# amoretti86/PSVO

Measured on AMD Instinct MI355X. Metric: particle-steps/sec, higher is better.
Workload: dtype f32

## Files before the change

psvo_amd/csrc/bsim_bwd2_impl.h:

```cpp
#pragma once
#define PSVO_BSIM_BWD_V2_UNIT 1
#include "bsim_bwd_impl.h"

namespace psvo {
PSVO_TIMERS_DEFINE(bsim_bwd2)

__device__ __forceinline__ float ldf(const float* base, unsigned off) {
    return *reinterpret_cast<const float*>(reinterpret_cast<const char*>(base) + off);
}
__device__ __forceinline__ int ldi(const int32_t* base, unsigned off) {
    return *reinterpret_cast<const int32_t*>(reinterpret_cast<const char*>(base) + off);
}
__device__ __forceinline__ void stf(float* base, unsigned off, float v) {
    *reinterpret_cast<float*>(reinterpret_cast<char*>(base) + off) = v;
}

__device__ __forceinline__ float swap_add32(float lo, float hi) {
    asm volatile("s_nop 1\n\tv_permlane32_swap_b32 %0, %1" : "+v"(lo), "+v"(hi));
    return lo + hi;
}
__device__ __forceinline__ float swap_add16(float lo, float hi) {
    asm volatile("s_nop 1\n\tv_permlane16_swap_b32 %0, %1" : "+v"(lo), "+v"(hi));
    return lo + hi;
}
// ... 132 lines not shown
        i_isig[d] = 1.f / a.isig[d];
        im[d] = a.imean[b * DX + d];
        mi[d] = a.minit[b * DX + d];
    }
    if constexpr (DX <= 2) {
        keep_in_vgpr(isf); keep_in_vgpr(rp); keep_in_vgpr(isfk); keep_in_vgpr(isg); keep_in_vgpr(ikap2);
        keep_in_vgpr(pc); keep_in_vgpr(pic); keep_in_vgpr(pi1); keep_in_vgpr(pi2);
    }
    const float ninf = -__builtin_huge_valf();
    const float aw = valid ? a.dscore[(size_t)b * N + n] : 0.f;

    const unsigned NM = (unsigned)N * M;
    unsigned o_nm = 4u * ((unsigned)b * NM + n * M + m);
    unsigned o_dnm[DX], o_knm[DY], o_dn[DX];
#pragma unroll
    for (int d = 0; d < DX; ++d) {
        o_dnm[d] = 4u * (((unsigned)b * DX + d) * NM + n * M + m);
        o_dn[d] = 4u * (((unsigned)b * DX + d) * N + n);
    }
#pragma unroll
    for (int k = 0; k < DY; ++k) o_knm[k] = 4u * (((unsigned)b * DY + k) * NM + n * M + m);
    unsigned o_n = 4u * ((unsigned)b * N + n);
    unsigned o_d = 4u * ((unsigned)b * DX), o_k = 4u * ((unsigned)b * DY);
    const unsigned s_nm = 4u * B * NM, s_dnm = s_nm * DX, s_knm = s_nm * DY, s_dn = 4u * B * DX * N, s_n = 4u * B * N,
                   s_d = 4u * B * DX, s_k = 4u * B * DY;

    float st[DX + 1], st_l = 0.f;
    int st_t = 0;
    auto put_slot = [&](float* buf, int j, const float (&raw)[DX + 1], float l) {
        float F[DX];
#pragma unroll
        for (int d = 0; d < DX; ++d) F[d] = raw[d] * rp[d];
        const float W = j < N ? (raw[DX] - l) * kLog2e : ninf;
        if constexpr (JM == 3) {
            const float Wf = fmaxf(W, -1e30f);
            uint4* q = reinterpret_cast<uint4*>(buf + j * PS);
            q[0] = bf16x3_b(F[0]);
            q[1] = bf16x3_b(F[DX > 1 ? 1 : 0]);
            q[2] = bf16x3_b(Wf - (F[0] * F[0] + F[DX > 1 ? 1 : 0] * F[DX > 1 ? 1 : 0]));
            q[3] = bf16x3_b(1.f);
            *reinterpret_cast<float4*>(buf + j * PS + 16) = make_float4(F[0], F[DX > 1 ? 1 : 0], 0.f, 0.f);
        } else if constexpr (JM == 2) {
            *reinterpret_cast<float4*>(buf + j * PS) = make_float4(F[0], F[1], W - (F[0] * F[0] + F[DX > 1 ? 1 : 0] * F[DX > 1 ? 1 : 0]), 1.f);
        } else if constexpr (DX <= 3) {
            float4 v;
            v.x = F[0];
            v.y = DX > 1 ? F[DX > 1 ? 1 : 0] : 0.f;
            v.z = DX > 2 ? F[DX > 2 ? 2 : 0] : 0.f;
            v.w = W;
            *reinterpret_cast<float4*>(buf + j * PS) = v;
        } else if constexpr (kSplitTile) {
            *reinterpret_cast<float4*>(buf + 4 * j) = make_float4(F[0], F[1], F[2], F[3]);
            buf[4 * NP + j] = W;
        } else {
            *reinterpret_cast<float4*>(buf + j * PS) = make_float4(F[0], F[1], F[2], F[3]);
            *reinterpret_cast<float4*>(buf + j * PS + 4) = make_float4(W, 0.f, 0.f, 0.f);
        }
    };
    auto tile_entry = [&](const float* buf, int j, float (&F)[DX], float& W) {
        if constexpr (kSplitTile) {
            const float4 e = *reinterpret_cast<const float4*>(buf + 4 * j);
            F[0] = e.x; F[DX > 1 ? 1 : 0] = e.y; F[DX > 2 ? 2 : 0] = e.z; F[DX > 3 ? 3 : 0] = e.w;
            W = buf[4 * NP + j];
        } else {
            read_slot<DX>(buf + j * PS, F, W);
        }
    };
    static_assert(offsetof(BsimBwdArgs, logW) - offsetof(BsimBwdArgs, Fm) == 8 &&
                  offsetof(BsimBwdArgs, lse) - offsetof(BsimBwdArgs, Fm) == 16 && offsetof(BsimBwdArgs, Fm) % 32 == 0,
                  "BsimBwdArgs: forward-tile pointer block");
    auto get_slot = [&](int tt, int j, float (&raw)[DX + 1], const float* Fm, const float* logW) {
        const unsigned tb = (unsigned)tt * B + b;
        const unsigned jc = j < N ? j : N - 1;
#pragma unroll
        for (int d = 0; d < DX; ++d) raw[d] = ldf(Fm, 4u * ((tb * DX + d) * N + jc));
        raw[DX] = ldf(logW, 4u * (tb * N + jc));
    };
    float st2[DX + 1];
    const bool two_slots = (DX >= 3) && NP > NTB;
    auto stage_load = [&](int tt) {
        unsigned long long pt[4];
        arg_block<4>((unsigned)offsetof(BsimBwdArgs, Fm), pt);
        st_t = tt;
        st_l = ldf(reinterpret_cast<const float*>(pt[2]), 4u * ((unsigned)tt * B + b));
        if (tid < NP) get_slot(tt, tid, st, reinterpret_cast<const float*>(pt[0]), reinterpret_cast<const float*>(pt[1]));
        if (two_slots && tid + NTB < NP)
            get_slot(tt, tid + NTB, st2, reinterpret_cast<const float*>(pt[0]), reinterpret_cast<const float*>(pt[1]));
    };
    auto stage_store = [&](float* buf) {
        if (tid < NP) put_slot(buf, tid, st, st_l);
        if (two_slots && tid + NTB < NP) put_slot(buf, tid + NTB, st2, st_l);
        for (int j = tid + (two_slots ? 2 : 1) * NTB; j < NP; j += NTB) {
            float raw[DX + 1];
            get_slot(st_t, j, raw, PSVO_ARG(BsimBwdArgs, Fm), PSVO_ARG(BsimBwdArgs, logW));
            put_slot(buf, j, raw, st_l);
        }
    };
    if (T >= 2) {
        stage_load(0);
        stage_store(tile);
    }
    __syncthreads();

    constexpr bool kAccLds = (DX >= 3);
    constexpr int kRowsA = 2 * DX + DY, kRowsB = 5 * DX, kSlotsB = 8;
    float acc[kAccLds ? 1 : AC::kN];
    float* const accA = red + 16 + wave * (kRowsA * 32 + kRowsB * kSlotsB);
    float* const accB = accA + kRowsA * 32;
    auto acc_is_lead = [](int k) { return k < 4 * DX || (k >= 5 * DX && k < 6 * DX); };
    auto acc_row = [](int k) {
        return k < 4 * DX ? k : k < 5 * DX ? k - 4 * DX : k < 6 * DX ? 4 * DX + (k - 5 * DX)
               : k < 7 * DX ? DX + (k - 6 * DX) : 2 * DX + (k - 7 * DX);
    };
    const int s32 = cl * M + m;
    if constexpr (kAccLds) {
        for (int i = lane; i < kRowsA * 32 + kRowsB * kSlotsB; i += 64) accA[i] = 0.f;
    } else {
#pragma unroll
        for (int i = 0; i < AC::kN; ++i) acc[i] = 0.f;
    }
    auto acc_add = [&](int k, float v) {
        if constexpr (kAccLds) {
            if (acc_is_lead(k)) atomicAdd(&accB[acc_row(k) * kSlotsB + cl], v);
            else atomicAdd(&accA[acc_row(k) * 32 + s32], v);
        } else {
            acc[k] += v;
        }
    };
    float dX[DX];
#pragma unroll
    for (int d = 0; d < DX; ++d) dX[d] = 0.f;

    struct StepIn {
        float eps[DX], bm[DX], xp[DX], mu1[DX], y[DY], om, lam2;
        int sel;
    };
    static_assert(offsetof(BsimBwdArgs, dscore) - offsetof(BsimBwdArgs, obs) == 56 && offsetof(BsimBwdArgs, obs) % 64 == 0 &&
                  offsetof(BsimBwdArgs, eps_b) - offsetof(BsimBwdArgs, obs) == 8 &&
                  offsetof(BsimBwdArgs, bwX) - offsetof(BsimBwdArgs, obs) == 16 &&
                  offsetof(BsimBwdArgs, sel) - offsetof(BsimBwdArgs, obs) == 24 &&
                  offsetof(BsimBwdArgs, lam2_all) - offsetof(BsimBwdArgs, obs) == 32 &&
                  offsetof(BsimBwdArgs, om_all) - offsetof(BsimBwdArgs, obs) == 40 &&
                  offsetof(BsimBwdArgs, mu1_all) - offsetof(BsimBwdArgs, obs) == 48, "BsimBwdArgs: input pointer block");
    auto load_step = [&](bool lst, bool fst, StepIn& s) {
        unsigned long long pb[8];
        arg_block<8>((unsigned)offsetof(BsimBwdArgs, obs), pb);
        const float* const p_obs = reinterpret_cast<const float*>(pb[0]);
        const float* const p_eps = reinterpret_cast<const float*>(pb[1]);
        const float* const p_bwX = reinterpret_cast<const float*>(pb[2]);
        const int32_t* const p_sel = reinterpret_cast<const int32_t*>(pb[3]);
        const float* const p_lam2 = reinterpret_cast<const float*>(pb[4]);
        const float* const p_om = reinterpret_cast<const float*>(pb[5]);
        const float* const p_mu1 = reinterpret_cast<const float*>(pb[6]);
        const float* const p_bm = PSVO_ARG(BsimBwdArgs, bmu2);
        s.sel = ldi(p_sel, o_n);
#pragma unroll
        for (int d = 0; d < DX; ++d) {
            s.eps[d] = ldf(p_eps, o_dnm[d]);
            s.bm[d] = ldf(p_bm, o_d + 4u * d);
            s.xp[d] = lst ? 0.f : ldf(p_bwX, o_dn[d] + s_dn);
            s.mu1[d] = lst ? 0.f : ldf(p_mu1, o_dn[d]);
        }
#pragma unroll
        for (int k = 0; k < DY; ++k) s.y[k] = ldf(p_obs, o_k + 4u * k);
        s.om = ldf(p_om, o_nm);
        s.lam2 = fst ? 0.f : ldf(p_lam2, o_nm);
    };
    auto advance = [&]() {
        o_nm += s_nm; o_n += s_n; o_d += s_d; o_k += s_k;
#pragma unroll
        for (int d = 0; d < DX; ++d) { o_dnm[d] += s_dnm; o_dn[d] += s_dn; }
#pragma unroll
        for (int k = 0; k < DY; ++k) o_knm[k] += s_knm;
    };
    StepIn cur_in, nxt_in;
    load_step(T == 1, true, cur_in);

    phase_skew(a.skew);
    SEC_INIT(bsim_bwd2)
    for (int t = 0; t < T; ++t) {
        SEC(0);
        const bool first = (t == 0), last = (t == T - 1);
        const float* cur = tile + ((t + 1) & 1) * NP * PS;
        float* nxt = tile + (t & 1) * NP * PS;
        constexpr bool kLateTile = (DX == 4);
        if (!kLateTile && t + 1 < T && t >= 1) stage_load(t);
        advance();
        constexpr bool kLatePrefetch = (DX >= 3);
        if (!kLatePrefetch && t + 1 < T) load_step(t + 2 == T, false, nxt_in);
        SEC(1);

        float xp[DX], eps[DX], bm[DX], mu1[DX], mu[DX], x[DX], y[DY];
        const int sel = cur_in.sel;
#pragma unroll
        for (int d = 0; d < DX; ++d) {
            eps[d] = cur_in.eps[d];
            bm[d] = cur_in.bm[d];
            xp[d] = cur_in.xp[d];
            mu1[d] = cur_in.mu1[d];
            if (!last) {
                mu[d] = pc[d] * fmaf(pi1[d], mu1[d], pi2[d] * bm[d]);
                x[d] = fmaf(pc[d], eps[d], mu[d]);
            } else {
                mu[d] = mi[d];
                x[d] = fmaf(s_init[d], eps[d], mu[d]);
            }
        }
#pragma unroll
        for (int k = 0; k < DY; ++k) y[k] = cur_in.y[k];
        const float pi_m = valid ? exp2_fast(cur_in.om * kLog2e) : 0.f;
        const float issel = (m == sel) ? 1.f : 0.f;
        const float dphi = aw * pi_m;
        const float dlam = -aw * (issel - pi_m);

        float dxt[DX];
#pragma unroll
        for (int d = 0; d < DX; ++d) dxt[d] = h0 ? issel * dX[d] : 0.f;

        SEC(2);
        if (!first) {
            if (h0) {
#pragma unroll
                for (int d = 0; d < DX; ++d) xw[d * CM + cl * M + m] = x[d] * rp[d];
                xw[DX * CM + cl * M + m] = cur_in.lam2;
                xw[(DX + 1) * CM + cl * M + m] = dlam;
            }
            __builtin_amdgcn_fence(__ATOMIC_RELEASE, "wavefront");
            __builtin_amdgcn_wave_barrier();
            __builtin_amdgcn_fence(__ATOMIC_ACQUIRE, "wavefront");

            if constexpr (RO) {
#pragma unroll 1
                for (int r = 0; r < 2; ++r) {
                    const int it4 = 4 * (4 * r + g);
                    f2 xa[DX], xb[DX], Ua[DX], Ub[DX], Va[DX], Vb[DX];
#pragma unroll
// ... 234 lines not shown
                    if (g == 0 || DX > 3) {
#pragma unroll
                        for (int jt = 0; jt < JC; ++jt) {
                            float F[DX], W;
                            read_slot<DX>(cbase + jt * 16 * PS, F, W);
                            (void)W;
                            const int j = (c * JC + jt) * 16 + j16;
                            if constexpr (DX <= 3) {
                                const float sc = D4[jt][DX];
#pragma unroll
                                for (int d = 0; d < DX; ++d) ja[d * NP + j] = D4[jt][d] - F[d] * sc;
                                ja[DX * NP + j] = sc;
                            } else {
                                const float sc = __shfl(D4[jt][0], 16 + j16);
                                if (g == 0) {
#pragma unroll
                                    for (int d = 0; d < DX; ++d) ja[d * NP + j] = D4[jt][d] - F[d] * sc;
                                    ja[DX * NP + j] = sc;
                                }
                            }
                        }
                    }
                }
            }
#pragma unroll
            for (int r = 0; r < 2; ++r) {
                float vv[4 * 2 * DX], o[UVS];
#pragma unroll
                for (int d = 0; d < DX; ++d) {
                    vv[0 * 2 * DX + d] = Ua[r][d].x; vv[1 * 2 * DX + d] = Ua[r][d].y;
                    vv[2 * 2 * DX + d] = Ub[r][d].x; vv[3 * 2 * DX + d] = Ub[r][d].y;
                    vv[0 * 2 * DX + DX + d] = Va[r][d].x; vv[1 * 2 * DX + DX + d] = Va[r][d].y;
                    vv[2 * 2 * DX + DX + d] = Vb[r][d].x; vv[3 * 2 * DX + DX + d] = Vb[r][d].y;
                }
                float red2[2 * DX];
                row_reduce_scatter<2 * DX>(vv, red2);
#pragma unroll
                for (int e = 0; e < UVS; ++e) o[e] = e < 2 * DX ? red2[e < 2 * DX ? e : 0] : 0.f;
                if ((j16 & 3) == 0) {
                    float* dst = uw + (4 * (4 * r + g) + (j16 >> 2)) * UVS;
#pragma unroll
                    for (int e = 0; e < UVS; e += 4)
                        *reinterpret_cast<float4*>(dst + e) = make_float4(o[e], o[e + 1], o[e + 2], o[e + 3]);
                }
            }
            }
            __builtin_amdgcn_fence(__ATOMIC_RELEASE, "wavefront");
            __builtin_amdgcn_wave_barrier();
            __builtin_amdgcn_fence(__ATOMIC_ACQUIRE, "wavefront");
            SEC(3);
            if (h0) {
                float uv[UVS];
#pragma unroll
                for (int e = 0; e < UVS; e += 4) {
                    const float4 q4 = *reinterpret_cast<const float4*>(uw + (cl * M + m) * UVS + e);
                    uv[e] = q4.x; uv[e + 1] = q4.y; uv[e + 2] = q4.z; uv[e + 3] = q4.w;
                }
                if constexpr (JM >= 2) {
#pragma unroll
                    for (int d = 0; d < DX; ++d) {
                        const float xs = x[d] * rp[d], r1 = uv[d], r2 = uv[DX + d];
                        uv[d] = xs - r1;
                        uv[DX + d] = fmaf(xs, xs - 2.f * r1, r2);
                    }
                }
#pragma unroll
                for (int d = 0; d < DX; ++d) {
                    dxt[d] -= dlam * uv[d] * isfk[d];
                    acc_add(AC::kSf + d, dlam * (uv[DX + d] * ikap2 - 1.f) * isf[d]);
                }
            }
        } else {
#pragma unroll
            for (int d = 0; d < DX; ++d) {
                const float z = (x[d] - im[d]) * i_isig[d];
                const float tz = dphi * z * i_isig[d];
                if (h0) {
                    dxt[d] -= tz;
                    acc_add(AC::kSiota + d, dphi * (z * z - 1.f) * i_isig[d]);
                }
            }
        }

        if (kLatePrefetch && t + 1 < T) load_step(t + 2 == T, false, nxt_in);
        if (kLateTile && t + 1 < T && t >= 1) stage_load(t);
        SEC(4);
        float dxp_part[DX];
#pragma unroll
        for (int d = 0; d < DX; ++d) dxp_part[d] = 0.f;
        {
            float dFo[DX];
#pragma unroll
            for (int d = 0; d < DX; ++d) dFo[d] = 0.f;
            if (!last) {
                float fmx[DX];
                MQ::template eval_part<PART>(wf, part, x, fmx);
#pragma unroll
                for (int d = 0; d < DX; ++d) fmx[d] += xor_lane<M>(fmx[d]);
#pragma unroll
                for (int d = 0; d < DX; ++d) {
                    const float z = (xp[d] - fmx[d]) * isf[d];
                    dFo[d] = dphi * z * isf[d];
                    if (h0) {
                        dxp_part[d] = -dFo[d];
                        acc_add(AC::kSf + d, dphi * (z * z - 1.f) * isf[d]);
                    }
                }
                MQ::template bwd_input_part<PART>(wf, part, x, dFo, dxt);
            }
            static_assert(offsetof(BsimBwdArgs, dFt) - offsetof(BsimBwdArgs, xt) == 8 &&
                          offsetof(BsimBwdArgs, dGt) - offsetof(BsimBwdArgs, xt) == 16 &&
                          offsetof(BsimBwdArgs, dmu1) - offsetof(BsimBwdArgs, xt) == 24 && offsetof(BsimBwdArgs, xt) % 32 == 0,
                          "BsimBwdArgs: row pointer block");
            unsigned long long pr[4];
            arg_block<4>((unsigned)offsetof(BsimBwdArgs, xt), pr);
            if (srow) {
#pragma unroll
                for (int d = 0; d < DX; ++d) {
                    stf(reinterpret_cast<float*>(pr[1]), o_dnm[d] - s_dnm, dFo[d]);
                    stf(reinterpret_cast<float*>(pr[0]), o_dnm[d] - s_dnm, x[d]);
                }
            }
            float gm[DY], dGo[DY];
            MG::template eval_part<PART>(wg, part, x, gm);
#pragma unroll
            for (int k = 0; k < DY; ++k) gm[k] += xor_lane<M>(gm[k]);
#pragma unroll
            for (int k = 0; k < DY; ++k) {
                float dmean = 1.f;
                if (a.emission) { dmean = emis_dmean(gm[k]); gm[k] = emis_mean(gm[k]); }
                const float z = (y[k] - gm[k]) * isg[k];
                dGo[k] = dphi * z * isg[k] * dmean;
                if (h0) acc_add(AC::kSg + k, dphi * (z * z - 1.f) * isg[k]);
                if (srow) stf(reinterpret_cast<float*>(pr[2]), o_knm[k] - s_knm, dGo[k]);
            }
            MG::template bwd_input_part<PART>(wg, part, x, dGo, dxt);
        }

        SEC(5);
        float dmu[DX], sce[DX], dxp[DX], dim[DX];
#pragma unroll
        for (int d = 0; d < DX; ++d) {
            const float v3 = (first && h0) ? dphi * (x[d] - im[d]) * i_isig[d] * i_isig[d] : 0.f;
            dmu[d] = group_sum<G>(dxt[d]);
            sce[d] = group_sum<G>(dxt[d] * eps[d]);
            dxp[d] = group_sum<G>(dxp_part[d]);
            dim[d] = first ? group_sum<G>(v3) : 0.f;
        }
        float outv[DX];
        if (!last) {
            float dmu1[DX];
#pragma unroll
            for (int d = 0; d < DX; ++d) {
                dmu1[d] = dmu[d] * pc[d] * pi1[d];
                outv[d] = dmu[d] * pc[d] * pi2[d];
                if (lead) {
                    stf(PSVO_ARG(BsimBwdArgs, dmu1), o_dn[d] - s_dn, dmu1[d]);
                    acc_add(AC::kSc + d, sce[d] + aw * pic[d]);
                    acc_add(AC::kSmm1 + d, dmu[d] * mu1[d]);
                    acc_add(AC::kSmb + d, dmu[d] * bm[d]);
                    acc_add(AC::kSmm + d, dmu[d] * mu[d]);
                }
            }
            {
                constexpr int kQS = (H / 4 < G) ? H / 4 : G;
                float dq[DX];
#pragma unroll
                for (int d = 0; d < DX; ++d) dq[d] = 0.f;
                MQ::template bwd_input_part<kQS>(wqi, (lane % G) & (kQS - 1), xp, dmu1, dq);
#pragma unroll
                for (int d = 0; d < DX; ++d) dxp[d] += group_sum<kQS>(dq[d]);
            }
        } else {
#pragma unroll
            for (int d = 0; d < DX; ++d) {
                outv[d] = dmu[d];
                if (lead) {
                    stf(PSVO_ARG(BsimBwdArgs, dmu1), o_dn[d] - s_dn, 0.f);
                    acc_add(AC::kSinit + d, sce[d] + aw * is_init[d]);
                }
            }
        }
#pragma unroll
        for (int d = 0; d < DX; ++d) dX[d] = dxp[d];
        if (lead) {
#pragma unroll
            for (int d = 0; d < DX; ++d) {
                stf(PSVO_ARG(BsimBwdArgs, dbmu2_rows), o_dn[d] - s_dn, last ? 0.f : outv[d]);
                if (last) PSVO_ARG(BsimBwdArgs, dminit_rows)[((size_t)b * DX + d) * N + n] = outv[d];
                if (first) PSVO_ARG(BsimBwdArgs, dimean_rows)[((size_t)b * DX + d) * N + n] = dim[d];
            }
        }
        SEC(6);
        __syncthreads();
        const size_t tb = (size_t)t * B + b;
        if (!first) {
            const size_t tbm = tb - B;
            float* const pF = PSVO_ARG(BsimBwdArgs, dFm_part) + (tbm * nblk + blk) * DX * N;
            float* const pW = PSVO_ARG(BsimBwdArgs, dlogW_part) + (tbm * nblk + blk) * N;
            for (int j = tid; j < N; j += NTB) {
#pragma unroll
                for (int d = 0; d < NA; ++d) {
                    const float* col = jacc + d * NP + j;
                    const float a0 = col[0], a1 = col[NA * NP], a2 = col[2 * NA * NP], a3 = col[3 * NA * NP];
                    const float s = (a0 + a1) + (a2 + a3);
                    if (d < DX) pF[d * N + j] = s * isfk[d < DX ? d : 0];
                    else pW[j] = s;
                }
            }
        }
        if (last) {
            float* const pF = PSVO_ARG(BsimBwdArgs, dFm_part) + (tb * nblk + blk) * DX * N;
            float* const pW = PSVO_ARG(BsimBwdArgs, dlogW_part) + (tb * nblk + blk) * N;
            for (int j = tid; j < N; j += NTB) {
#pragma unroll
                for (int d = 0; d < DX; ++d) pF[d * N + j] = 0.f;
                pW[j] = 0.f;
            }
        }
        SEC(7);
        if (t + 1 < T && t >= 1) stage_store(nxt);
        cur_in = nxt_in;
        __syncthreads();
        SEC(8);
    }

    for (int i = 0; i < AC::kN; ++i) {
        float v = 0.f;
        if constexpr (kAccLds) {
            if (acc_is_lead(i)) v = lane < kSlotsB ? accB[acc_row(i) * kSlotsB + lane] : 0.f;
            else v = lane < 32 ? accA[acc_row(i) * 32 + lane] : 0.f;
        } else {
#pragma unroll
            for (int k = 0; k < AC::kN; ++k) v = (k == i) ? acc[k] : v;
        }
        v = wave_sum(v);
        if (lane == 0) red[wave] = v;
        __syncthreads();
        if (tid == 0) {
            float s = 0.f;
            for (int w = 0; w < nwv; ++w) s += red[w];
            a.sacc_part[((size_t)b * nblk + blk) * AC::kN + i] = s;
        }
        __syncthreads();
    }
}

static inline void bsim2_geometry(int N, int M, int& cpb, int& nblk) {
    cpb = 4 * (64 / (2 * M));
    nblk = (N + cpb - 1) / cpb;
}

static inline bool bsim2_supported(int B, int T, int N, int M, int Dx, int Dy) {
    if (!(M == 4 || M == 8 || M == 16 || M == 32)) return false;
    const long long big = (long long)T * B * (Dx > Dy ? Dx : Dy) * N * M * 4;
    return big < (1ll << 32);
}

template <int DX, int DY, int H, int M>
static int launch_bsim_bwd2(const BsimBwdArgs& a, const BsimBwdOut& o, int jm, hipStream_t stream) {
    using MQ = MlpLds<DX, H, DX, 1>;
    using MG = MlpLds<DX, H, DY, 1>;
    const int PS = (jm == 3 && DX == 2) ? 20 : (DX == 4) ? 5 : BTileSlot<DX>::kFloats;
    constexpr int UVS = (2 * DX + 3) & ~3;
    int cpb, nblk;
    bsim2_geometry(a.N, M, cpb, nblk);
    const int NP = ((a.N + 127) / 128) * 128;
    const size_t lds = sizeof(float) * (2 * MQ::kSize + MG::kSize + 2 * (size_t)NP * PS + 4 * (size_t)(DX + 1) * NP +
                                        4 * (DX + 2) * 32 + 4 * 32 * UVS + 16 +
                                        (DX >= 3 ? 4 * ((2 * DX + DY) * 32 + 5 * DX * 8) : 0));
    if (lds > 160 * 1024) return PSVO_ERR_UNSUPPORTED;
    BsimBwdArgs as = a;
    as.skew = (int)(2560.0 * NP / 128.0 * (3 * DX + 4) / 10.0 * g_tune_skew_pct / 100.0);
    clear_hip_error();
    if (jm == 3 && DX == 2) {
        if constexpr (DX == 2)
            hipLaunchKernelGGL((bsim_bwd2_kernel<DX, DY, H, M, 3>), dim3(nblk, a.B), dim3(256), lds, stream, as);
    } else if (jm == 2 && DX == 2) {
        if constexpr (DX == 2)
            hipLaunchKernelGGL((bsim_bwd2_kernel<DX, DY, H, M, 2>), dim3(nblk, a.B), dim3(256), lds, stream, as);
    } else if (jm == 1 && DX == 2) {
        if constexpr (DX == 2)
            hipLaunchKernelGGL((bsim_bwd2_kernel<DX, DY, H, M, 1>), dim3(nblk, a.B), dim3(256), lds, stream, as);
    } else {
        hipLaunchKernelGGL((bsim_bwd2_kernel<DX, DY, H, M, 0>), dim3(nblk, a.B), dim3(256), lds, stream, as);
    }
    (void)o;
    return launch_status();
}

template <int DX, int DY, int H>
static int bb2_dispatch_m(const BsimBwdArgs& a, const BsimBwdOut& o, int M, int jm, hipStream_t s) {
    switch (M) {
        case 4: return launch_bsim_bwd2<DX, DY, H, 4>(a, o, jm, s);
        case 8: return launch_bsim_bwd2<DX, DY, H, 8>(a, o, jm, s);
        case 16: return launch_bsim_bwd2<DX, DY, H, 16>(a, o, jm, s);
        case 32: return launch_bsim_bwd2<DX, DY, H, 32>(a, o, jm, s);
        default: return PSVO_ERR_UNSUPPORTED;
    }
}

template <int DX, int DY>
static int bb2_dispatch_h(const BsimBwdArgs& a, const BsimBwdOut& o, int H, int M, int jm, hipStream_t s) {
    switch (H) {
        case 16: return bb2_dispatch_m<DX, DY, 16>(a, o, M, jm, s);
// ... 17 lines not shown
```

psvo_amd/csrc/bsim_fwd.hip:

```cpp
#include "common.h"

namespace psvo {
inline namespace PSVO_LNS {
PSVO_TIMERS_DEFINE(bsim_fwd)


struct BsimArgs {
    int B, T, N;
    int emission;
    psvo_mlp f, g, q1inv;
    const float *X, *Fm, *logW, *lse;
    const float *sig_f, *sig_g, *sig_q1inv, *sig_bq2;
    const float *bmu2, *minit, *sig_init, *imean, *isig;
    const float *obs, *eps_b, *u_b;
    const int32_t* sel_in;
    float *bwX, *flp, *glp, *Omega;
    int32_t* sel_out;
    float* score;
    float *lam2_all, *om_all, *mu1_all;
};

template <int DX>
struct TileSlot {
    static constexpr int kFloats = (DX <= 3) ? 4 : 8;
// ... 84 lines not shown
    const float ninf = -__builtin_huge_valf();

    float st[kMaxStage][DX + 1], st_l = 0.f;
    auto stage_load = [&](int tt) {
        const size_t tb = (size_t)tt * B + b;
        st_l = a.lse[tb];
#pragma unroll
        for (int r = 0; r < kMaxStage; ++r) {
            const int j = tid + r * NTB;
            if (j < NP) {
                const int jc = j < N ? j : N - 1;
#pragma unroll
                for (int d = 0; d < DX; ++d) st[r][d] = a.Fm[(tb * DX + d) * N + jc];
                st[r][DX] = a.logW[tb * N + jc];
            }
        }
    };
    auto stage_store = [&](float* buf) {
#pragma unroll
        for (int r = 0; r < kMaxStage; ++r) {
            const int j = tid + r * NTB;
            if (j < NP) {
                float F[DX];
#pragma unroll
                for (int d = 0; d < DX; ++d) F[d] = st[r][d] * rp[d];
                const float W = j < N ? (st[r][DX] - st_l) * kLog2e : ninf;
                if constexpr (DX <= 3) {
                    float4 v;
                    v.x = F[0];
                    v.y = DX > 1 ? F[DX > 1 ? 1 : 0] : 0.f;
                    v.z = DX > 2 ? F[DX > 2 ? 2 : 0] : 0.f;
                    v.w = W;
                    *reinterpret_cast<float4*>(buf + j * PS) = v;
                } else {
                    *reinterpret_cast<float4*>(buf + j * PS) = make_float4(F[0], F[1], F[2], F[3]);
                    *reinterpret_cast<float4*>(buf + j * PS + 4) = make_float4(W, 0.f, 0.f, 0.f);
                }
            }
        }
    };

    if (T >= 2) {
        stage_load(T - 2);
        stage_store(tile);
    }

    float eps_c[DX], bmu_c[DX], obs_c[DY], u_c = 0.f;
    int sel_c = 0;
    auto load_inputs = [&](int t, float (&e)[DX], float (&bm)[DX], float (&o)[DY], float& uu, int& ss) {
        const size_t tb = (size_t)t * B + b;
#pragma unroll
        for (int d = 0; d < DX; ++d) {
            e[d] = a.eps_b[((tb * DX + d) * N + n) * M + m];
            bm[d] = a.bmu2[tb * DX + d];
        }
#pragma unroll
        for (int k = 0; k < DY; ++k) o[k] = a.obs[tb * DY + k];
        if (a.sel_in) ss = a.sel_in[tb * N + n];
        else uu = a.u_b[tb * N + n];
    };
    load_inputs(T - 1, eps_c, bmu_c, obs_c, u_c, sel_c);
    __syncthreads();

    float xp[DX];
#pragma unroll
    for (int d = 0; d < DX; ++d) xp[d] = 0.f;
    float score = 0.f;

    SEC_INIT(bsim_fwd)
    auto step = [&](auto last_tag, auto zero_tag, const int t) {
        SEC(0);
        const size_t tb = (size_t)t * B + b;
        const float* cur = tile + ((T - 1 - t) & 1) * NP * PS;
        float* nxt = tile + ((T - t) & 1) * NP * PS;
        const bool last = last_tag;
        const bool tzero = zero_tag;

        float eps_n[DX], bmu_n[DX], obs_n[DY], u_n = 0.f;
        int sel_n = 0;
        if (!tzero) load_inputs(t - 1, eps_n, bmu_n, obs_n, u_n, sel_n);
        if (t >= 2) stage_load(t - 2);

        SEC(1);
        float x[DX], q_lp;
        if (last) {
            float mu[DX];
#pragma unroll
            for (int d = 0; d < DX; ++d) {
                mu[d] = mi[d];
                x[d] = fmaf(s_init[d], eps_c[d], mu[d]);
            }
            q_lp = diag_lp<DX>(x, mu, is_init, kinit);
            if (a.mu1_all && valid && lead) {
#pragma unroll
                for (int d = 0; d < DX; ++d) a.mu1_all[(tb * DX + d) * N + n] = 0.f;
            }
        } else {
            float m1[DX], mu[DX];
            {
                constexpr int kQS = (H / 4 < G) ? H / 4 : G;
                MQ::template eval_part<kQS>(wqi, (tid % G) & (kQS - 1), xp, m1);
#pragma unroll
                for (int d = 0; d < DX; ++d) m1[d] = group_sum<kQS>(m1[d]);
            }
            if (a.mu1_all && valid && lead) {
#pragma unroll
                for (int d = 0; d < DX; ++d) a.mu1_all[(tb * DX + d) * N + n] = m1[d];
            }
#pragma unroll
            for (int d = 0; d < DX; ++d) {
                mu[d] = pc[d] * fmaf(pi1[d], m1[d], pi2[d] * bmu_c[d]);
                x[d] = fmaf(pc[d], eps_c[d], mu[d]);
            }
            q_lp = diag_lp<DX>(x, mu, pic, kq);
        }

        SEC(2);
        float phi = 0.f;
        if (!last) {
            float fmx[DX];
            if constexpr (HS == 1) {
                MQ::template eval<kRolled>(wf, x, fmx);
            } else {
                MQ::template eval_part<HS, ilog2(M)>(wf, hpart, x, fmx);
#pragma unroll
                for (int d = 0; d < DX; ++d) fmx[d] += xor_lane<M>(fmx[d]);
            }
            phi = diag_lp<DX>(xp, fmx, isf, kf);
        }
        float gm[DY];
        if constexpr (HS == 1) {
            MG::template eval<kRolled>(wg, x, gm);
        } else {
            MG::template eval_part<HS, ilog2(M)>(wg, hpart, x, gm);
#pragma unroll
            for (int k = 0; k < DY; ++k) gm[k] += xor_lane<M>(gm[k]);
        }
        if (a.emission) {
#pragma unroll
            for (int k = 0; k < DY; ++k) gm[k] = emis_mean(gm[k]);
        }
        const float g_lp = diag_lp<DY>(obs_c, gm, isg, kg);

        SEC(3);
        float lam;
        if (!tzero) {
            float xq[4][DX];
#pragma unroll
            for (int d = 0; d < DX; ++d) {
                float t4[4];
                quad_bcast4(x[d] * rp[d], t4);
#pragma unroll
                for (int i = 0; i < 4; ++i) xq[i][d] = t4[i];
            }
            f2 xa[DX], xb[DX];
#pragma unroll
            for (int d = 0; d < DX; ++d) {
                xa[d] = f2{xq[0][d], xq[1][d]};
                xb[d] = f2{xq[2][d], xq[3][d]};
            }
            f2 mxa = f2{ninf, ninf}, mxb = mxa, sma = f2{0.f, 0.f}, smb = sma;
            const int nqh = (NP >> 2) / HS;
            const int j0 = hpart * nqh;
            auto block = [&](auto jb_tag, int k0) {
                constexpr int JB = decltype(jb_tag)::value;
                f2 va[JB], vb[JB];
                f2 bma = f2{ninf, ninf}, bmb = bma;
#pragma unroll
                for (int c = 0; c < JB; ++c) {
                    const float* p = cur + ((j0 + k0 + c) * 4 + q) * PS;
                    float F[DX], W;
                    if constexpr (DX <= 3) {
                        const float4 sl = *reinterpret_cast<const float4*>(p);
                        F[0] = sl.x;
                        if (DX > 1) F[DX > 1 ? 1 : 0] = sl.y;
                        if (DX > 2) F[DX > 2 ? 2 : 0] = sl.z;
                        W = sl.w;
                    } else {
                        const float4 sl = *reinterpret_cast<const float4*>(p);
                        F[0] = sl.x; F[1] = sl.y; F[2] = sl.z; F[3] = sl.w;
                        W = p[4];
                    }
                    f2 la = f2{W, W}, lb = la;
#pragma unroll
                    for (int d = 0; d < DX; ++d) {
                        const f2 Fd = f2{F[d], F[d]};
                        const f2 ua = xa[d] - Fd, ub = xb[d] - Fd;
                        la = pk_fma(-ua, ua, la);
                        lb = pk_fma(-ub, ub, lb);
                    }
                    va[c] = la;
                    vb[c] = lb;
                    bma = pk_max(bma, la);
                    bmb = pk_max(bmb, lb);
                }
                const f2 nma = pk_max(mxa, bma), nmb = pk_max(mxb, bmb);
                const f2 ba = f2{nma.x == ninf ? 0.f : nma.x, nma.y == ninf ? 0.f : nma.y};
                const f2 bb = f2{nmb.x == ninf ? 0.f : nmb.x, nmb.y == ninf ? 0.f : nmb.y};
                const f2 ra = mxa - ba, rb = mxb - bb;
                sma = sma * f2{exp2_fast(ra.x), exp2_fast(ra.y)};
                smb = smb * f2{exp2_fast(rb.x), exp2_fast(rb.y)};
#pragma unroll
                for (int c = 0; c < JB; ++c) {
                    const f2 da = va[c] - ba, db = vb[c] - bb;
                    sma += f2{exp2_fast(da.x), exp2_fast(da.y)};
                    smb += f2{exp2_fast(db.x), exp2_fast(db.y)};
                }
                mxa = nma;
                mxb = nmb;
            };
            int k0 = 0;
            for (; k0 + 16 <= nqh; k0 += 16) block(std::integral_constant<int, 16>{}, k0);
            if (nqh - k0 >= 8) {
                block(std::integral_constant<int, 8>{}, k0);
                k0 += 8;
            }
            if (nqh - k0 >= 4) block(std::integral_constant<int, 4>{}, k0);
            SEC(4);
            const float mx[4] = {mxa.x, mxa.y, mxb.x, mxb.y};
            const float sm[4] = {sma.x, sma.y, smb.x, smb.y};
            float lm = ninf, ls = 0.f;
#pragma unroll
            for (int i = 0; i < 4; ++i) {
                float gm = fmaxf(mx[i], xor_lane<1>(mx[i]));
                gm = fmaxf(gm, xor_lane<2>(gm));
                if constexpr (HS == 2) gm = fmaxf(gm, xor_lane<M>(gm));
                const float base = (gm == ninf) ? 0.f : gm;
                float sc = sm[i] * exp2_fast(mx[i] - base);
                sc += xor_lane<1>(sc);
                sc += xor_lane<2>(sc);
                if constexpr (HS == 2) sc += xor_lane<M>(sc);
                if (i == q) {
                    lm = gm;
                    ls = sc;
                }
            }
            const float lam2 = lm + log2_fast(ls);
            lam = fmaf(kLn2, lam2, kf);
            if (a.lam2_all && valid && hpart == 0) a.lam2_all[(tb * N + n) * M + m] = lam2;
        } else {
            lam = diag_lp<DX>(x, im, i_isig, kiota);
        }

        SEC(5);
        const float om_raw = lam + phi + g_lp - q_lp;
        const float omx = group_max<M>(om_raw);
        const float pw = exp2_fast((om_raw - omx) * kLog2e);
        const float cdfv = group_incl_scan<M>(pw, m);
        const float total = __shfl(cdfv, gbase + M - 1);
        const float omega = om_raw - fmaf(kLn2, log2_fast(total), omx);
        if (a.om_all && valid && hpart == 0) a.om_all[(tb * N + n) * M + m] = omega;
        int sel;
        if (a.sel_in) {
            sel = sel_c;
        } else {
            const unsigned long long bal = __ballot(cdfv <= u_c * total);
            const unsigned long long mask = (M == 64) ? ~0ull : (((1ull << M) - 1ull) << gbase);
            sel = min((int)__popcll(bal & mask), M - 1);
        }
        const int src = gbase + sel;
        float xs[DX];
#pragma unroll
        for (int d = 0; d < DX; ++d) xs[d] = __shfl(x[d], src);
        const float om_s = __shfl(omega, src);
        const float phi_s = __shfl(phi, src);
        SEC(6);
        const float g_s = __shfl(g_lp, src);
        const float q_s = __shfl(q_lp, src);
        const float lam_s = __shfl(lam, src);
        const float Om = om_s + q_s + logM;

        if (valid && lead) {
#pragma unroll
            for (int d = 0; d < DX; ++d) a.bwX[(tb * DX + d) * N + n] = xs[d];
            a.glp[tb * N + n] = g_s;
            a.Omega[tb * N + n] = Om;
            a.sel_out[tb * N + n] = sel;
            if (!last) a.flp[(tb + B) * N + n] = phi_s;
            if (tzero) a.flp[(size_t)b * N + n] = lam_s;
        }
        score += g_s - Om + (last ? 0.f : phi_s) + (tzero ? lam_s : 0.f);

#pragma unroll
        for (int d = 0; d < DX; ++d) {
            xp[d] = xs[d];
            eps_c[d] = eps_n[d];
            bmu_c[d] = bmu_n[d];
        }
#pragma unroll
        for (int k = 0; k < DY; ++k) obs_c[k] = obs_n[k];
        u_c = u_n;
        sel_c = sel_n;

        SEC(7);
        if (t >= 2) stage_store(nxt);
        __syncthreads();
        SEC(8);
    };
    if constexpr (kPeel) {
        step(std::true_type{}, std::false_type{}, T - 1);
        for (int t = T - 2; t >= 1; --t) step(std::false_type{}, std::false_type{}, t);
        step(std::false_type{}, std::true_type{}, 0);
    } else {
        for (int t = T - 1; t >= 0; --t) step(t == T - 1, t == 0, t);
    }
    if (valid && lead) a.score[(size_t)b * N + n] = score;
}

template <int DX, int DY, int H, int M>
static int launch_bsim(const BsimArgs& a, hipStream_t stream) {
    using MQ = MlpLds<DX, H, DX, PSVO_L>;
    using MG = MlpLds<DX, H, DY, PSVO_L>;
    constexpr int PS = TileSlot<DX>::kFloats;
    const long long waves1 = ((long long)a.B * a.N * M + 63) / 64;
    const int HS = (waves1 < 2048 && 2 * M <= 64 && (H / 2) % 4 == 0 && (PSVO_L == 1 || g_tune_l2_split)) ? 2 : 1;
    const int NP = ((a.N + 16 * HS - 1) / (16 * HS)) * (16 * HS);
    int NTB = ((a.N * M * HS + 63) / 64) * 64;
    if (NTB > 256) NTB = 256;
    const int cpb = NTB / (M * HS);
    const size_t lds = sizeof(float) * (2 * MQ::kSize + MG::kSize + 2 * (size_t)NP * PS);
    dim3 grid((a.N + cpb - 1) / cpb, a.B);
    clear_hip_error();
    if (HS == 2) {
        if constexpr (2 * M <= 64 && (H / 2) % 4 == 0)
            hipLaunchKernelGGL((bsim_fwd_kernel<DX, DY, H, M, 2>), grid, dim3(NTB), lds, stream, a);
    } else {
        hipLaunchKernelGGL((bsim_fwd_kernel<DX, DY, H, M, 1>), grid, dim3(NTB), lds, stream, a);
    }
    return launch_status();
}

template <int DX, int DY, int H>
static int bsim_dispatch_m(const BsimArgs& a, int M, hipStream_t s) {
    switch (M) {
        case 4: return launch_bsim<DX, DY, H, 4>(a, s);
        case 8: return launch_bsim<DX, DY, H, 8>(a, s);
        case 16: return launch_bsim<DX, DY, H, 16>(a, s);
        case 32: return launch_bsim<DX, DY, H, 32>(a, s);
        default: return PSVO_ERR_UNSUPPORTED;
    }
}

template <int DX, int DY>
static int bsim_dispatch_h(const BsimArgs& a, int H, int M, hipStream_t s) {
    switch (H) {
#if PSVO_L == 1
        case 16: return bsim_dispatch_m<DX, DY, 16>(a, M, s);
#endif
        case 32: return bsim_dispatch_m<DX, DY, 32>(a, M, s);
        case 64: return bsim_dispatch_m<DX, DY, 64>(a, M, s);
        default: return PSVO_ERR_UNSUPPORTED;
    }
}

template <int DX>
static int bsim_dispatch_dy(const BsimArgs& a, int Dy, int H, int M, hipStream_t s) {
    switch (Dy) {
        case 1: return bsim_dispatch_h<DX, 1>(a, H, M, s);
        case 2: return bsim_dispatch_h<DX, 2>(a, H, M, s);
        default: return PSVO_ERR_UNSUPPORTED;
    }
}

}
}

PSVO_L2_DECL(psvo_bsim_forward)
PSVO_ENTRY(psvo_bsim_forward)(const psvo_desc* desc, const float* X, const float* Fm, const float* logW,
                                 const float* lse, const psvo_mlp* f, const psvo_mlp* g, const psvo_mlp* q1_inv,
                                 const float* sig_f, const float* sig_g, const float* sig_q1inv,
                                 const float* sig_bq2, const float* bmu2, const float* minit,
                                 const float* sig_init, const float* imean, const float* isig, const float* obs,
                                 const float* eps_b, const float* u_b, const int32_t* sel_in, float* bwX,
                                 float* flp, float* glp, float* Omega, int32_t* sel_out, float* score,
                                 float* lam2_all, float* om_all, float* mu1_all,
                                 void* stream) {
    using namespace psvo;
    if (!desc_layers_ok(desc)) return PSVO_ERR_UNSUPPORTED;
// ... 34 lines not shown
```

psvo_amd/csrc/common.h:

```cpp
#pragma once
#include <cstddef>
#include <type_traits>
#include <hip/hip_runtime.h>
#include <stdint.h>

#include "../../include/psvo_hip.h"

#ifndef PSVO_L
#define PSVO_L 1
#endif
#if PSVO_L == 1
#define PSVO_LNS l1
#define PSVO_ENTRY(name) extern "C" int name
#define PSVO_L2_DECL(name) extern "C" __attribute__((visibility("hidden"))) decltype(name) name##_l2;
#elif PSVO_L == 2
#define PSVO_LNS l2
#define PSVO_ENTRY(name) extern "C" __attribute__((visibility("hidden"))) int name##_l2
#define PSVO_L2_DECL(name)
#else
#error "PSVO_L must be 1 or 2"
#endif

namespace psvo {

// ... 6 lines not shown
inline void clear_hip_error() { (void)hipGetLastError(); }
inline int launch_status() {
    const hipError_t e = hipGetLastError();
    if (e != hipSuccess) g_last_hip_error = e;
    return e == hipSuccess ? PSVO_OK : PSVO_ERR_HIP;
}

inline bool desc_layers_ok(const psvo_desc* d) { return !d || (d->layers >= 0 && d->layers <= 2); }

extern int g_tune_l2_split;
extern int g_tune_filter_bwd_scan;

extern int g_tune_skew_pct;

__device__ __forceinline__ void phase_skew(int cycles) {
    unsigned hw;
    asm volatile("s_getreg_b32 %0, hwreg(HW_REG_HW_ID)" : "=s"(hw));
    if (cycles > 0 && ((hw >> 16) & 1u)) {
        for (int i = 0; i < cycles; i += 64 * 32) __builtin_amdgcn_s_sleep(32);
    }
}

inline bool mlp_layers_ok(const psvo_mlp* m) { return PSVO_L == 1 || !m || (m->Wh && m->bh); }

static inline int wr_cluster(int B, int N, int M) {
    int K = 8;
    while (K > 1 && ((long long)B * K > 256 || N < 4 * K || (N + K - 1) / K * (K - 1) >= N)) K >>= 1;
    (void)M;
    return K;
}

#ifdef PSVO_SECTION_TIMERS
#define PSVO_TIMERS_DEFINE(name)                                                                        \
    __device__ unsigned long long g_sec_##name[32];                                                       \
    extern "C" int psvo_debug_timers_##name(unsigned long long* out, int reset) {                         \
        if (hipMemcpyFromSymbol(out, HIP_SYMBOL(g_sec_##name), 32 * sizeof(unsigned long long)) != hipSuccess) \
            return -1;                                                                                    \
        if (reset) {                                                                                      \
            unsigned long long z[32] = {0};                                                               \
            if (hipMemcpyToSymbol(HIP_SYMBOL(g_sec_##name), z, sizeof(z)) != hipSuccess) return -1;       \
        }                                                                                                 \
        return 0;                                                                                         \
    }
#define SEC_INIT(name)                                                                          \
    unsigned long long* const _sec = g_sec_##name;                                              \
    const bool _rec = (blockIdx.x == 0 && blockIdx.y == 0 && threadIdx.x == 0);                 \
    unsigned long long _tp = clock64();
#define SEC(i)                                   \
    do {                                         \
        const unsigned long long _tn = clock64(); \
        if (_rec) _sec[i] += _tn - _tp;          \
        _tp = _tn;                               \
    } while (0)
#else
#define PSVO_TIMERS_DEFINE(name)
#define SEC_INIT(name)
#define SEC(i)
#endif

__device__ __forceinline__ float exp2_fast(float x) { return __builtin_amdgcn_exp2f(x); }
__device__ __forceinline__ float log2_fast(float x) { return __builtin_amdgcn_logf(x); }

typedef float f2 __attribute__((ext_vector_type(2)));
__device__ __forceinline__ f2 pk_fma(f2 a, f2 b, f2 c) { return __builtin_elementwise_fma(a, b, c); }
__device__ __forceinline__ f2 pk_max(f2 a, f2 b) { return __builtin_elementwise_max(a, b); }
template <int HALF>
__device__ __forceinline__ f2 pk_fma_bcast(f2 a, f2 b, f2 c) {
    f2 d;
    if constexpr (HALF == 0)
        asm("v_pk_fma_f32 %0, %1, %2, %3 op_sel_hi:[0,1,1]" : "=v"(d) : "v"(a), "v"(b), "v"(c));
    else
        asm("v_pk_fma_f32 %0, %1, %2, %3 op_sel:[1,0,0] op_sel_hi:[1,1,1]" : "=v"(d) : "v"(a), "v"(b), "v"(c));
    return d;
}

__device__ __forceinline__ void keep_in_vgpr(float& x) { asm volatile("" : "+v"(x)); }
template <int K>
__device__ __forceinline__ void keep_in_vgpr(float (&x)[K]) {
#pragma unroll
    for (int i = 0; i < K; ++i) asm volatile("" : "+v"(x[i]));
}

template <class T>
__device__ __forceinline__ T* arg_ptr(unsigned byte_off) {
    asm volatile("" : "+s"(byte_off));
    typedef const char __attribute__((address_space(4))) * kptr;
    const kptr kp = (kptr)__builtin_amdgcn_kernarg_segment_ptr();
    typedef T* const __attribute__((address_space(4))) * pptr;
    return *(pptr)(kp + byte_off);
}
template <int NPTR>
__device__ __forceinline__ void arg_block(unsigned byte_off, unsigned long long (&out)[NPTR]) {
    static_assert(NPTR == 2 || NPTR == 4 || NPTR == 8, "pointer block of 2, 4 or 8");
    asm volatile("" : "+s"(byte_off));
    typedef const char __attribute__((address_space(4))) * kptr;
    const kptr kp = (kptr)__builtin_amdgcn_kernarg_segment_ptr();
    typedef unsigned long long vec_t __attribute__((ext_vector_type(NPTR)));
    typedef const vec_t __attribute__((address_space(4))) * vptr;
    const vec_t v = *(vptr)(kp + byte_off);
#pragma unroll
    for (int i = 0; i < NPTR; ++i) out[i] = v[i];
}
#define PSVO_ARG(args_type, field) \
    ::psvo::arg_ptr<std::remove_pointer_t<decltype(args_type::field)>>((unsigned)offsetof(args_type, field))

__device__ __forceinline__ float emis_mean(float r) { return (r > 20.f ? r : log1pf(expf(r))) + 1e-6f; }
__device__ __forceinline__ float emis_dmean(float r) { return 1.f / (1.f + expf(-r)); }

template <int DIN, int H, int DOUT, int L = 1>
struct MlpLds;

template <int DIN, int H, int DOUT>
struct MlpLds<DIN, H, DOUT, 1> {
    static constexpr int kW1 = 0;
    static constexpr int kB1 = DIN * H;
    static constexpr int kW2 = kB1 + H;
    static constexpr int kB2 = kW2 + DOUT * H;
    static constexpr int kSize = kB2 + ((DOUT + 3) & ~3);

    __device__ static void load(float* __restrict__ w, const psvo_mlp& p, int tid, int nthreads) {
        for (int i = tid; i < DIN * H; i += nthreads) w[kW1 + i] = p.W1[i];
        for (int i = tid; i < H; i += nthreads) w[kB1 + i] = p.b1[i];
        for (int i = tid; i < DOUT * H; i += nthreads) {
            const int o = i / H, k = i - o * H;
            w[kW2 + i] = p.W2[k * DOUT + o];
        }
        for (int i = tid; i < ((DOUT + 3) & ~3); i += nthreads) w[kB2 + i] = i < DOUT ? p.b2[i] : 0.f;
    }

    __device__ __forceinline__ static void group4(const float* __restrict__ w, int k, const float (&x)[DIN],
                                                  f2 (&acc)[DOUT]) {
        const float4 b = *reinterpret_cast<const float4*>(w + kB1 + k);
        f2 ha = f2{b.x, b.y}, hb = f2{b.z, b.w};
#pragma unroll
        for (int i = 0; i < DIN; ++i) {
            const float4 wi = *reinterpret_cast<const float4*>(w + kW1 + i * H + k);
            const f2 xi = f2{x[i], x[i]};
            ha = pk_fma(xi, f2{wi.x, wi.y}, ha);
            hb = pk_fma(xi, f2{wi.z, wi.w}, hb);
        }
        const f2 zero = f2{0.f, 0.f};
        ha = pk_max(ha, zero);
        hb = pk_max(hb, zero);
#pragma unroll
        for (int o = 0; o < DOUT; ++o) {
            const float4 wo = *reinterpret_cast<const float4*>(w + kW2 + o * H + k);
            acc[o] = pk_fma(ha, f2{wo.x, wo.y}, acc[o]);
            acc[o] = pk_fma(hb, f2{wo.z, wo.w}, acc[o]);
        }
    }

    template <bool ROLLED = false>
    __device__ __forceinline__ static void eval(const float* __restrict__ w, const float (&x)[DIN],
                                                float (&out)[DOUT]) {
        f2 acc[DOUT];
#pragma unroll
        for (int o = 0; o < DOUT; ++o) acc[o] = f2{w[kB2 + o], 0.f};
        if constexpr (ROLLED && (H % 8 == 0) && (H > 8)) {
#pragma unroll 1
            for (int k = 0; k < H; k += 8) {
                group4(w, k, x, acc);
                group4(w, k + 4, x, acc);
            }
        } else {
#pragma unroll
            for (int k = 0; k < H; k += 4) group4(w, k, x, acc);
        }
#pragma unroll
        for (int o = 0; o < DOUT; ++o) out[o] = acc[o].x + acc[o].y;
    }

    template <int S, int PB = 0>
// ... 425 lines not shown
```

Measured before the change: 241.1 million.

## Tag kernel-arg pointers as global and move tile staging store earlier

Pointers read from the kernel-argument block are now cast through the global address space, so the compiler can emit global loads and stores instead of generic flat ones. The backward and forward simulation steps also move the LDS tile store and the swap of next-step inputs ("take over") earlier in the step, ahead of the late compute, to overlap latency with the remaining work before the barrier. The forward kernel keeps copies of u and sel for the current step so the early swap does not corrupt resampling, and pins the swapped registers in VGPRs. The cost is extra register pressure from values held live across more of the step.

Result: faster. 245.9 million, median of 6 (+2.0%).

```diff
diff --git a/psvo_amd/csrc/bsim_bwd2_impl.h b/psvo_amd/csrc/bsim_bwd2_impl.h
--- a/psvo_amd/csrc/bsim_bwd2_impl.h
+++ b/psvo_amd/csrc/bsim_bwd2_impl.h
@@ -238,10 +238,10 @@
         unsigned long long pt[4];
         arg_block<4>((unsigned)offsetof(BsimBwdArgs, Fm), pt);
         st_t = tt;
-        st_l = ldf(reinterpret_cast<const float*>(pt[2]), 4u * ((unsigned)tt * B + b));
-        if (tid < NP) get_slot(tt, tid, st, reinterpret_cast<const float*>(pt[0]), reinterpret_cast<const float*>(pt[1]));
+        st_l = ldf(as_global<const float>(pt[2]), 4u * ((unsigned)tt * B + b));
+        if (tid < NP) get_slot(tt, tid, st, as_global<const float>(pt[0]), as_global<const float>(pt[1]));
         if (two_slots && tid + NTB < NP)
-            get_slot(tt, tid + NTB, st2, reinterpret_cast<const float*>(pt[0]), reinterpret_cast<const float*>(pt[1]));
+            get_slot(tt, tid + NTB, st2, as_global<const float>(pt[0]), as_global<const float>(pt[1]));
     };
     auto stage_store = [&](float* buf) {
         if (tid < NP) put_slot(buf, tid, st, st_l);
@@ -301,13 +301,13 @@
     auto load_step = [&](bool lst, bool fst, StepIn& s) {
         unsigned long long pb[8];
         arg_block<8>((unsigned)offsetof(BsimBwdArgs, obs), pb);
-        const float* const p_obs = reinterpret_cast<const float*>(pb[0]);
-        const float* const p_eps = reinterpret_cast<const float*>(pb[1]);
-        const float* const p_bwX = reinterpret_cast<const float*>(pb[2]);
-        const int32_t* const p_sel = reinterpret_cast<const int32_t*>(pb[3]);
-        const float* const p_lam2 = reinterpret_cast<const float*>(pb[4]);
-        const float* const p_om = reinterpret_cast<const float*>(pb[5]);
-        const float* const p_mu1 = reinterpret_cast<const float*>(pb[6]);
+        const float* const p_obs = as_global<const float>(pb[0]);
+        const float* const p_eps = as_global<const float>(pb[1]);
+        const float* const p_bwX = as_global<const float>(pb[2]);
+        const int32_t* const p_sel = as_global<const int32_t>(pb[3]);
+        const float* const p_lam2 = as_global<const float>(pb[4]);
+        const float* const p_om = as_global<const float>(pb[5]);
+        const float* const p_mu1 = as_global<const float>(pb[6]);
         const float* const p_bm = PSVO_ARG(BsimBwdArgs, bmu2);
         s.sel = ldi(p_sel, o_n);
 #pragma unroll
@@ -708,6 +708,12 @@
             }
         }
 
+        constexpr bool kEarlyTakeOver = !kLatePrefetch;
+        auto take_over = [&]() {
+            if (t + 1 < T && t >= 1) stage_store(nxt);
+            cur_in = nxt_in;
+        };
+        if (kEarlyTakeOver) take_over();
         if (kLatePrefetch && t + 1 < T) load_step(t + 2 == T, false, nxt_in);
         if (kLateTile && t + 1 < T && t >= 1) stage_load(t);
         SEC(4);
@@ -743,8 +749,8 @@
             if (srow) {
 #pragma unroll
                 for (int d = 0; d < DX; ++d) {
-                    stf(reinterpret_cast<float*>(pr[1]), o_dnm[d] - s_dnm, dFo[d]);
-                    stf(reinterpret_cast<float*>(pr[0]), o_dnm[d] - s_dnm, x[d]);
+                    stf(as_global<float>(pr[1]), o_dnm[d] - s_dnm, dFo[d]);
+                    stf(as_global<float>(pr[0]), o_dnm[d] - s_dnm, x[d]);
                 }
             }
             float gm[DY], dGo[DY];
@@ -758,7 +764,7 @@
                 const float z = (y[k] - gm[k]) * isg[k];
                 dGo[k] = dphi * z * isg[k] * dmean;
                 if (h0) acc_add(AC::kSg + k, dphi * (z * z - 1.f) * isg[k]);
-                if (srow) stf(reinterpret_cast<float*>(pr[2]), o_knm[k] - s_knm, dGo[k]);
+                if (srow) stf(as_global<float>(pr[2]), o_knm[k] - s_knm, dGo[k]);
             }
             MG::template bwd_input_part<PART>(wg, part, x, dGo, dxt);
         }
@@ -818,6 +824,7 @@
             }
         }
         SEC(6);
+        if (!kEarlyTakeOver) take_over();
         __syncthreads();
         const size_t tb = (size_t)t * B + b;
         if (!first) {
@@ -845,8 +852,6 @@
             }
         }
         SEC(7);
-        if (t + 1 < T && t >= 1) stage_store(nxt);
-        cur_in = nxt_in;
         __syncthreads();
         SEC(8);
     }
diff --git a/psvo_amd/csrc/bsim_fwd.hip b/psvo_amd/csrc/bsim_fwd.hip
--- a/psvo_amd/csrc/bsim_fwd.hip
+++ b/psvo_amd/csrc/bsim_fwd.hip
@@ -190,6 +190,25 @@
         if (t >= 2) stage_load(t - 2);
 
         SEC(1);
+        constexpr bool kEarlyTakeOver = kPeel;
+        const float u_t = u_c;
+        const int sel_t = sel_c;
+        auto take_over = [&]() {
+            if (t >= 2) stage_store(nxt);
+#pragma unroll
+            for (int d = 0; d < DX; ++d) {
+                eps_c[d] = eps_n[d];
+                bmu_c[d] = bmu_n[d];
+            }
+#pragma unroll
+            for (int k = 0; k < DY; ++k) obs_c[k] = obs_n[k];
+            u_c = u_n;
+            sel_c = sel_n;
+            if constexpr (kEarlyTakeOver) {
+                keep_in_vgpr(eps_c); keep_in_vgpr(bmu_c); keep_in_vgpr(obs_c); keep_in_vgpr(u_c);
+                asm volatile("" : "+v"(sel_c));
+            }
+        };
         float x[DX], q_lp;
         if (last) {
             float mu[DX];
@@ -325,6 +344,7 @@
             }
             if (nqh - k0 >= 4) block(std::integral_constant<int, 4>{}, k0);
             SEC(4);
+            if constexpr (kEarlyTakeOver) take_over();
             const float mx[4] = {mxa.x, mxa.y, mxb.x, mxb.y};
             const float sm[4] = {sma.x, sma.y, smb.x, smb.y};
             float lm = ninf, ls = 0.f;
@@ -360,9 +380,9 @@
         if (a.om_all && valid && hpart == 0) a.om_all[(tb * N + n) * M + m] = omega;
         int sel;
         if (a.sel_in) {
-            sel = sel_c;
+            sel = sel_t;
         } else {
-            const unsigned long long bal = __ballot(cdfv <= u_c * total);
+            const unsigned long long bal = __ballot(cdfv <= u_t * total);
             const unsigned long long mask = (M == 64) ? ~0ull : (((1ull << M) - 1ull) << gbase);
             sel = min((int)__popcll(bal & mask), M - 1);
         }
@@ -388,20 +408,11 @@
             if (tzero) a.flp[(size_t)b * N + n] = lam_s;
         }
         score += g_s - Om + (last ? 0.f : phi_s) + (tzero ? lam_s : 0.f);
-
-#pragma unroll
-        for (int d = 0; d < DX; ++d) {
-            xp[d] = xs[d];
-            eps_c[d] = eps_n[d];
-            bmu_c[d] = bmu_n[d];
-        }
-#pragma unroll
-        for (int k = 0; k < DY; ++k) obs_c[k] = obs_n[k];
-        u_c = u_n;
-        sel_c = sel_n;
+#pragma unroll
+        for (int d = 0; d < DX; ++d) xp[d] = xs[d];
 
         SEC(7);
-        if (t >= 2) stage_store(nxt);
+        if constexpr (!kEarlyTakeOver) take_over();
         __syncthreads();
         SEC(8);
     };
diff --git a/psvo_amd/csrc/common.h b/psvo_amd/csrc/common.h
--- a/psvo_amd/csrc/common.h
+++ b/psvo_amd/csrc/common.h
@@ -112,12 +112,18 @@
 }
 
 template <class T>
+using global_ptr = T __attribute__((address_space(1))) *;
+template <class T>
+__device__ __forceinline__ T* as_global(unsigned long long bits) {
+    return (T*)(global_ptr<T>)bits;
+}
+template <class T>
 __device__ __forceinline__ T* arg_ptr(unsigned byte_off) {
     asm volatile("" : "+s"(byte_off));
     typedef const char __attribute__((address_space(4))) * kptr;
     const kptr kp = (kptr)__builtin_amdgcn_kernarg_segment_ptr();
-    typedef T* const __attribute__((address_space(4))) * pptr;
-    return *(pptr)(kp + byte_off);
+    typedef const global_ptr<T> __attribute__((address_space(4))) * pptr;
+    return (T*)*(pptr)(kp + byte_off);
 }
 template <int NPTR>
 __device__ __forceinline__ void arg_block(unsigned byte_off, unsigned long long (&out)[NPTR]) {
```
